# rubengooj/stvo-pl

Measured on AMD Instinct MI355X. Metric: stereo frames/s (match+optimizePose), higher is better.
Workload: dtype u8/fp4+f64; 1 GPU; BASELINE configs[2]: KITTI-00-shaped stereo with points + lines (ORB + LBD rows), grid-windowed stereo match (points and lines) + f2f brute-force mutual-NNR match (points and lines) + full GN optimizePose (config_kitti.yaml), device-resident per-frame pipeline; the streams cycle through the 8 sequence ids / 3 KITTI calibrations of configs[4] (sequence s on rank s mod G); streams_per_gpu=3072, parallelism=seq-shard x1

## Files before the change

### stvo-pl_amd/csrc/pose_block.h

```cpp
#pragma once
#include <type_traits>

#include "kernels.h"
#include "pose_math.h"

namespace stvo {

namespace {

constexpr int ACT_CONTINUE = 0, ACT_BREAK = 1, ACT_FAIL = 2;

struct PoseSh {
    double DT[16];
    double DT0[16];
    double DT1[16];
    double DTr[16];
    double cov[36];
    double eig[6];
    double H[36];
    double g[6];
    double err, err_prev, err_out, lambda;
    double s_p, s_l;
    unsigned long long xchg[2];
    int action, good, n_inl_p, n_inl_l, n_m_p, n_m_l, evals, itmp;
};

__device__ __forceinline__ void store_total(PoseSh* sh, int k, double s) {
    if (k < 21) {
        const int i = (k >= 6) + (k >= 11) + (k >= 15) + (k >= 18) + (k >= 20), j = k - (i * (13 - i)) / 2 + i;
        sh->H[i * 6 + j] = s;
        sh->H[j * 6 + i] = s;
    } else if (k < 27) {
        sh->g[k - 21] = s;
    } else {
        sh->err = s / (double)(sh->n_inl_l + sh->n_inl_p);
    }
}

template <int NWORK>
struct BlockOps {
    static constexpr int NW = NWORK;
    static constexpr int WTHREADS = NWORK * 64;

    template <int CTRL, int ROW_MASK>
    static __device__ __forceinline__ double dpp_add(double v) {
        const long long b = __double_as_longlong(v);
        const int lo = __builtin_amdgcn_update_dpp(0, (int)(b & 0xFFFFFFFFll), CTRL, ROW_MASK, 0xf, true);
        const int hi = __builtin_amdgcn_update_dpp(0, (int)(b >> 32), CTRL, ROW_MASK, 0xf, true);
        return v + __longlong_as_double(((long long)hi << 32) | (unsigned long long)(unsigned)lo);
    }
    static __device__ __forceinline__ double wave_sum_lane63(double v) {
        v = dpp_add<0x111, 0xf>(v);
        v = dpp_add<0x112, 0xf>(v);
        v = dpp_add<0x114, 0xf>(v);
        v = dpp_add<0x118, 0xf>(v);
        v = dpp_add<0x142, 0xa>(v);
        v = dpp_add<0x143, 0xc>(v);
        return v;
    }
    static __device__ __forceinline__ double wave_sum(double v) {
#pragma unroll
        for (int off = 32; off > 0; off >>= 1) v += __shfl_xor(v, off, 64);
        return v;
    }
    static __device__ __forceinline__ int wave_sum_i(int v) {
#pragma unroll
        for (int off = 32; off > 0; off >>= 1) v += __shfl_xor(v, off, 64);
        return v;
    }

    static __device__ __forceinline__ double fold32(double a, double b) {
        const unsigned long long ab = (unsigned long long)__double_as_longlong(a), bb = (unsigned long long)__double_as_longlong(b);
        const auto lo = __builtin_amdgcn_permlane32_swap((unsigned)ab, (unsigned)bb, false, false);
        const auto hi = __builtin_amdgcn_permlane32_swap((unsigned)(ab >> 32), (unsigned)(bb >> 32), false, false);
        return __longlong_as_double((long long)(((unsigned long long)hi[0] << 32) | lo[0])) +
               __longlong_as_double((long long)(((unsigned long long)hi[1] << 32) | lo[1]));
    }
    static __device__ __forceinline__ double fold16(double a, double b) {
        const unsigned long long ab = (unsigned long long)__double_as_longlong(a), bb = (unsigned long long)__double_as_longlong(b);
        const auto lo = __builtin_amdgcn_permlane16_swap((unsigned)ab, (unsigned)bb, false, false);
        const auto hi = __builtin_amdgcn_permlane16_swap((unsigned)(ab >> 32), (unsigned)(bb >> 32), false, false);
        return __longlong_as_double((long long)(((unsigned long long)hi[0] << 32) | lo[0])) +
               __longlong_as_double((long long)(((unsigned long long)hi[1] << 32) | lo[1]));
    }

    template <bool W>
    static __device__ __forceinline__ void sum28_fold(double* acc, double (*red)[28], bool sc = false) {
        const int lane = threadIdx.x & 63, wv = W ? (int)(threadIdx.x >> 6) : NW;
        if (W || sc) {
            double s14[14], s7[7];
#pragma unroll
            for (int k = 0; k < 14; ++k) s14[k] = fold32(acc[k], acc[14 + k]);
// ... 39 lines not shown
            }
        }
        __syncthreads();
#pragma unroll
        for (int k = 0; k < N; ++k) {
            double s = red[0][k];
#pragma unroll
            for (int w = 1; w < NW; ++w) s += red[w][k];
            out[k] = s;
        }
        __syncthreads();
    }

    template <bool W>
    static __device__ __forceinline__ int sum_int(int v, int* ired, bool sc = false) {
        const int lane = threadIdx.x & 63, wv = W ? (int)(threadIdx.x >> 6) : NW;
        if (W || sc) {
            const int s = wave_sum_i(v);
            if (lane == 0) ired[wv] = s;
        }
        __syncthreads();
        int t = 0;
#pragma unroll
        for (int w = 0; w < NW; ++w) t += ired[w];
        if (sc) t += ired[NW];
        __syncthreads();
        return t;
    }

    template <bool W>
    static __device__ __forceinline__ void sum_int4(const int* v, double (*red)[28], int* out, bool sc = false) {
        const int lane = threadIdx.x & 63, wv = W ? (int)(threadIdx.x >> 6) : NW;
        if (W || sc) {
#pragma unroll
            for (int k = 0; k < 4; ++k) {
                const int t = wave_sum_i(v[k]);
                if (lane == 0) reinterpret_cast<int*>(&red[wv][0])[k] = t;
            }
        }
        __syncthreads();
#pragma unroll
        for (int k = 0; k < 4; ++k) {
            int t = 0;
#pragma unroll
            for (int w = 0; w < NW; ++w) t += reinterpret_cast<const int*>(&red[w][0])[k];
            if (sc) t += reinterpret_cast<const int*>(&red[NW][0])[k];
            out[k] = t;
        }
    }

    static constexpr int HIST_W = 260;
    static constexpr int SEL_HW = 64, SEL_PART = 6 * SEL_HW;
    static_assert(SEL_PART * 4 % 8 == 0 && SEL_PART + 8 * (NWORK + 1) <= 2 * HIST_W, "selection scratch");

    static __device__ __forceinline__ int wave_incl_scan_i(int v) {
        v += __builtin_amdgcn_update_dpp(0, v, 0x111, 0xf, 0xf, true);
        v += __builtin_amdgcn_update_dpp(0, v, 0x112, 0xf, 0xf, true);
        v += __builtin_amdgcn_update_dpp(0, v, 0x114, 0xf, 0xf, true);
        v += __builtin_amdgcn_update_dpp(0, v, 0x118, 0xf, 0xf, true);
        v += __builtin_amdgcn_update_dpp(0, v, 0x142, 0xa, 0xf, true);
        v += __builtin_amdgcn_update_dpp(0, v, 0x143, 0xc, 0xf, true);
        return v;
    }
    static __device__ __forceinline__ void sel_scan(const unsigned* h, int kk, int& bin, int& below, int& cnt) {
        const int lane = threadIdx.x & 63;
        const unsigned w = h[lane];
        const int c0 = (int)(w & 0xFFFFu), c1 = (int)(w >> 16), sum = c0 + c1;
        const int incl = wave_incl_scan_i(sum), excl = incl - sum;
        const unsigned long long hit = __ballot(excl <= kk && kk < incl);
        const int L = hit ? __builtin_ctzll(hit) : 0;
        const bool up = kk >= excl + c0;
        bin = __builtin_amdgcn_readlane(2 * lane + (up ? 1 : 0), L);
        below = __builtin_amdgcn_readlane(excl + (up ? c0 : 0), L);
        cnt = __builtin_amdgcn_readlane(up ? c1 : c0, L);
    }
    template <int N, typename K, typename KeyFn>
    static __device__ __forceinline__ void sel_and_or(KeyFn&& key, unsigned mask, unsigned long long* part) {
        K k_and = ~(K)0, k_or = 0;
#pragma unroll
        for (int k = 0; k < N; ++k)
            if ((mask >> k) & 1u) {
                const K kv = key(k);
                k_and &= kv;
                k_or |= kv;
            }
        auto dpp_step = [&](auto ctrl_c, auto rmask_c) {
            constexpr int CTRL = decltype(ctrl_c)::value, RM = decltype(rmask_c)::value;
            const unsigned alo = (unsigned)k_and, ahi = (unsigned)((unsigned long long)k_and >> 32);
            const unsigned olo = (unsigned)k_or, ohi = (unsigned)((unsigned long long)k_or >> 32);
            const unsigned a0 = (unsigned)__builtin_amdgcn_update_dpp((int)alo, (int)alo, CTRL, RM, 0xf, false);
            const unsigned a1 = (unsigned)__builtin_amdgcn_update_dpp((int)ahi, (int)ahi, CTRL, RM, 0xf, false);
            const unsigned o0 = (unsigned)__builtin_amdgcn_update_dpp((int)olo, (int)olo, CTRL, RM, 0xf, false);
            const unsigned o1 = (unsigned)__builtin_amdgcn_update_dpp((int)ohi, (int)ohi, CTRL, RM, 0xf, false);
            k_and &= (K)(((unsigned long long)a1 << 32) | a0);
            k_or |= (K)(((unsigned long long)o1 << 32) | o0);
        };
        using std::integral_constant;
        dpp_step(integral_constant<int, 0x111>{}, integral_constant<int, 0xf>{});
        dpp_step(integral_constant<int, 0x112>{}, integral_constant<int, 0xf>{});
        dpp_step(integral_constant<int, 0x114>{}, integral_constant<int, 0xf>{});
        dpp_step(integral_constant<int, 0x118>{}, integral_constant<int, 0xf>{});
        dpp_step(integral_constant<int, 0x142>{}, integral_constant<int, 0xa>{});
        dpp_step(integral_constant<int, 0x143>{}, integral_constant<int, 0xc>{});
        if ((threadIdx.x & 63) == 63) {
            part[0] = (unsigned long long)k_and;
            part[1] = (unsigned long long)k_or;
        }
    }

    template <int NA, int NB, bool W, typename K, int BITS, typename KeyA, typename KeyB>
    static __device__ __forceinline__ void select2(KeyA&& ka, unsigned ma, int ktha, bool acta, KeyB&& kb, unsigned mb, int kthb, bool actb,
                                                   unsigned* S, unsigned long long* xchg, int& rot, K& outa, K& outb, bool sc = false) {
        static_assert(BITS == 32 || BITS == 64, "32- or 64-bit keys");
        const int tid = threadIdx.x, wv = tid >> 6;
        const bool own_b = W ? !sc : sc;
        constexpr bool PFA = BITS == 64 && NA >= 8, PFB = BITS == 64 && NB >= 8;
        K anda = 0, ora = ~(K)0, andb = 0, orb = ~(K)0;
        if (PFA || PFB) {
            unsigned long long* part = reinterpret_cast<unsigned long long*>(S + SEL_PART);
            if (W) {
                if (PFA) sel_and_or<NA, K>(ka, ma, part + 4 * wv);
                if (PFB && !sc) sel_and_or<NB, K>(kb, mb, part + 4 * wv + 2);
            }
            __syncthreads();
            unsigned long long a0 = ~0ull, o0 = 0ull, a1 = ~0ull, o1 = 0ull;
#pragma unroll
            for (int w = 0; w < NWORK; ++w) {
                if (PFA) { a0 &= part[4 * w]; o0 |= part[4 * w + 1]; }
                if (PFB) { a1 &= part[4 * w + 2]; o1 |= part[4 * w + 3]; }
            }
            if (PFA) { anda = (K)a0; ora = (K)o0; }
            if (PFB && !sc) { andb = (K)a1; orb = (K)o1; }
        }
        auto top_bit = [](K differ) -> int {
            return differ == 0 ? -1 : (BITS - 1) - (BITS == 64 ? __clzll((unsigned long long)differ) : __clz((unsigned)differ));
        };
        K pa = anda, pb = andb;
        int kka = ktha, kkb = kthb;
        int hia = acta ? top_bit(anda ^ ora) : -1, hib = actb ? top_bit(andb ^ orb) : -1;
        bool penda = false, pendb = false;
        auto count = [&](auto n_c, auto&& key, unsigned mask, K prefix, int hi, int lo, unsigned* h) {
            constexpr int N = decltype(n_c)::value;
#pragma unroll
            for (int k = 0; k < N; ++k) {
                const K kv = key(k);
                const K diff = kv ^ prefix;
                const bool same = hi + 1 >= BITS ? true : (diff >> (hi + 1 >= BITS ? 0 : hi + 1)) == 0;
                const unsigned bin = (unsigned)((kv >> lo) & 127);
                if (((mask >> k) & 1u) && same) atomicAdd(&h[bin >> 1], 1u << (16 * (bin & 1u)));
            }
        };
        auto decide = [&](auto n_c, bool own, auto&& key, unsigned mask, const unsigned* h, K& prefix, int& kk, int& hi, int lo, bool& pend,
                          unsigned long long* mail) {
            constexpr int N = decltype(n_c)::value;
            int bin, below, cnt;
            sel_scan(h, kk, bin, below, cnt);
            prefix = (prefix & ~((K)127 << lo)) | ((K)bin << lo);
            kk -= below;
            hi = lo - 1;
            if (cnt == 1 && lo > 0) {
                if (own) {
#pragma unroll
                    for (int k = 0; k < N; ++k) {
                        const K kv = key(k);
                        if (((mask >> k) & 1u) && ((kv ^ prefix) >> lo) == 0) *mail = (unsigned long long)kv;
                    }
                }
                pend = true;
                hi = -1;
            }
        };
        using std::integral_constant;
        while (hia >= 0 || hib >= 0) {
            const int loa = hia >= 6 ? hia - 6 : 0, lob = hib >= 6 ? hib - 6 : 0;
            unsigned* const ha = S + rot * SEL_HW;
            unsigned* const hb = S + (3 + rot) * SEL_HW;
            if (W && hia >= 0) count(integral_constant<int, NA>{}, ka, ma, pa, hia, loa, ha);
            if (own_b && hib >= 0) count(integral_constant<int, NB>{}, kb, mb, pb, hib, lob, hb);
            __syncthreads();
            if (W && tid < 2 * SEL_HW) {
                const int rc = rot == 0 ? 2 : rot - 1;
                S[((tid >> 6) * 3 + rc) * SEL_HW + (tid & 63)] = 0u;
            }
            if (hia >= 0) decide(integral_constant<int, NA>{}, W, ka, ma, ha, pa, kka, hia, loa, penda, xchg);
            if (hib >= 0) decide(integral_constant<int, NB>{}, own_b, kb, mb, hb, pb, kkb, hib, lob, pendb, xchg + 1);
            rot = rot == 2 ? 0 : rot + 1;
        }
        __syncthreads();
        if (penda) pa = (K)xchg[0];
        if (pendb) pb = (K)xchg[1];
        if (acta) outa = pa;
        if (actb) outb = pb;
    }

    template <int NA, int NB, bool W>
    static __device__ __forceinline__ void mad_sigma2(const double* va, unsigned ma, int na, const double* vb, unsigned mb, int nb, unsigned* S,
                                                      unsigned long long* xchg, int& rot, double& sa, double& sb, bool sc = false) {
        sa = 0.0;
        sb = 0.0;
        const bool acta = na != 0, actb = nb != 0;
        if (!acta && !actb) return;
        auto image = [](double v) -> unsigned long long {
            const unsigned long long b = (unsigned long long)__double_as_longlong(v);
            return (b >> 63) ? ~b : (b | 0x8000000000000000ull);
        };
        auto value = [](unsigned long long k) -> double {
            return __longlong_as_double((long long)((k >> 63) ? (k & 0x7FFFFFFFFFFFFFFFull) : ~k));
        };
        unsigned long long ra = 0ull, rb = 0ull;
        select2<NA, NB, W, unsigned long long, 64>([&](int k) { return image(va[k]); }, ma, na / 2, acta, [&](int k) { return image(vb[k]); }, mb,
                                                   nb / 2, actb, S, xchg, rot, ra, rb, sc);
        const double meda = value(ra), medb = value(rb);
        unsigned qa = 0u, qb = 0u;
        select2<NA, NB, W, unsigned, 32>([&](int k) { return __float_as_uint(fabsf((float)(va[k] - meda))); }, ma, na / 2, acta,
                                         [&](int k) { return __float_as_uint(fabsf((float)(vb[k] - medb))); }, mb, nb / 2, actb, S, xchg, rot, qa, qb, sc);
        if (acta) sa = 1.4826 * (double)__uint_as_float(qa);
        if (actb) sb = 1.4826 * (double)__uint_as_float(qb);
    }

    template <int N, bool W>
    static __device__ __forceinline__ void sum_at(const double* v, double (*red)[28], int slot0, double* out, bool sc = false) {
        const int lane = threadIdx.x & 63, wv = W ? (int)(threadIdx.x >> 6) : NW;
        if (W || sc) {
#pragma unroll
            for (int k = 0; k < N; ++k) {
                const double s = wave_sum_lane63(v[k]);
                if (lane == 63) red[wv][slot0 + k] = s;
            }
        }
        __syncthreads();
#pragma unroll
        for (int k = 0; k < N; ++k) {
            double s = red[0][slot0 + k];
#pragma unroll
            for (int w = 1; w < NW; ++w) s += red[w][slot0 + k];
            if (sc) s += red[NW][slot0 + k];
            out[k] = s;
        }
    }

    template <int NA, int NB, bool W>
    static __device__ __forceinline__ void outlier_cut(const double* ra, unsigned ma, int na, bool do_a, const double* rb, unsigned mb, int nb,
                                                       bool do_b, double inlier_k, unsigned& inla, unsigned& inlb, unsigned* S,
                                                       unsigned long long* xchg, int& rot, double (*red)[28], int* cnt, bool sc = false) {
        const bool own_b = W ? !sc : sc;
        double sa, sb;
        mad_sigma2<NA, NB, W>(ra, do_a ? ma : 0u, do_a ? na : 0, rb, do_b ? mb : 0u, do_b ? nb : 0, S, xchg, rot, sa, sb, sc);
        double v[6] = {0.0, 0.0, 0.0, 0.0, 0.0, 0.0};
        if (W) {
#pragma unroll
            for (int k = 0; k < NA; ++k)
                if (do_a && ((ma >> k) & 1u)) {
                    if (ra[k] < 2.0 * sa) {
                        v[0] += ra[k];
                        v[1] += 1.0;
                    }
                    v[2] += ra[k];
                }
        }
        if (own_b) {
#pragma unroll
            for (int k = 0; k < NB; ++k)
                if (do_b && ((mb >> k) & 1u)) {
                    if (rb[k] < 2.0 * sb) {
                        v[3] += rb[k];
                        v[4] += 1.0;
                    }
                    v[5] += rb[k];
// ... 147 lines not shown
#pragma unroll
        for (int i = 0; i < 16; ++i) DT[i] = sh->DT[i];
        pm::step_pose(DT, inc);
#pragma unroll
        for (int i = 0; i < 16; ++i) sh->DT[i] = DT[i];
    }
    if (norm3(inc) < min_error_change && norm3(inc + 3) < min_error_change) {
        sh->action = ACT_BREAK;
        return;
    }
    sh->err_prev = err;
    sh->action = ACT_CONTINUE;
}

__device__ __forceinline__ void t0_cov_from_H(PoseSh* sh, double* ws) {
    double H[36], Hi[36];
#pragma unroll
    for (int i = 0; i < 36; ++i) H[i] = sh->H[i];
    if (pm::inverse6_spd(H, Hi)) {
#pragma unroll
        for (int i = 0; i < 36; ++i) sh->cov[i] = Hi[i];
    } else {
#pragma unroll 1
        for (int i = 0; i < 36; ++i) ws[i] = sh->H[i];
        pm::inverse6_mem(ws, sh->cov);
    }
}

__device__ __forceinline__ void t0_is_good(PoseSh* sh, const double* DT, double err) {
    double C[36], w[6];
#pragma unroll
    for (int i = 0; i < 36; ++i) C[i] = sh->cov[i];
    pm::eig6_ql(C, w);
#pragma unroll
    for (int i = 0; i < 6; ++i) sh->eig[i] = w[i];
    sh->good = pm::is_good_solution(DT, w, err) ? 1 : 0;
}

__device__ __forceinline__ void t0_is_good_fast(PoseSh* sh, const double* DT, double err) {
    if (err < 0.0 || err > 1.0 || !pm::all_finite16(DT)) {
        sh->good = 0;
        return;
    }
    double C[36];
#pragma unroll
    for (int i = 0; i < 36; ++i) C[i] = sh->cov[i];
    if (pm::spd_unit_certificate(C) == 1) {
        sh->good = 1;
        return;
    }
    t0_is_good(sh, DT, err);
}

__device__ __forceinline__ void t0_commit(PoseSh* sh, stvo_pose_result* out, int status, int path, int it0, int it1, bool lazy_eig = false,
                                          double* next_T = nullptr) {
    bool eig_pending = false;
    if (lazy_eig) {
        double C[36];
#pragma unroll
        for (int i = 0; i < 36; ++i) C[i] = sh->cov[i];
        if (sh->err_out < 0.0 || sh->err_out > 1.0 || !pm::all_finite16(sh->DT)) {
            sh->good = 0;
        } else if (pm::spd_unit_certificate(C) == 1) {
            sh->good = 1;
            eig_pending = true;
        } else {
            t0_is_good(sh, sh->DT, sh->err_out);
        }
    } else {
        t0_is_good(sh, sh->DT, sh->err_out);
    }
    double DT[16];
#pragma unroll
    for (int i = 0; i < 16; ++i) {
        DT[i] = sh->DT[i];
        out->T_opt[i] = DT[i];
    }
    out->err_opt = sh->err_out;
    if (sh->good && !pm::is_identity16(DT)) {
        double Ti[16], x[6], T[16];
        pm::inverse_se3(DT, Ti);
        pm::logmap_se3(Ti, x);
        pm::expmap_se3(x, T);
#pragma unroll
        for (int i = 0; i < 16; ++i) out->T[i] = T[i];
        if (next_T) {
            const bool fin = pm::all_finite16(T);
#pragma unroll
            for (int i = 0; i < 16; ++i) next_T[i] = fin ? T[i] : ((i % 5 == 0) ? 1.0 : 0.0);
        }
#pragma unroll
        for (int i = 0; i < 36; ++i) out->cov[i] = sh->cov[i];
#pragma unroll
        for (int i = 0; i < 6; ++i) out->cov_eig[i] = eig_pending ? 0.0 : sh->eig[i];
        if (eig_pending) path |= PATH_EIG_PENDING;
        out->err = sh->err_out;
    } else {
#pragma unroll
        for (int i = 0; i < 16; ++i) out->T[i] = (i % 5 == 0) ? 1.0 : 0.0;
        if (next_T) {
#pragma unroll
            for (int i = 0; i < 16; ++i) next_T[i] = (i % 5 == 0) ? 1.0 : 0.0;
        }
#pragma unroll
        for (int i = 0; i < 36; ++i) out->cov[i] = 0.0;
#pragma unroll
        for (int i = 0; i < 6; ++i) out->cov_eig[i] = 0.0;
        out->err = -1.0;
        if (status == STVO_POSE_OK) status = STVO_POSE_REJECTED;
    }
    out->status = status;
    out->path = path;
    out->iters[0] = it0;
    out->iters[1] = it1;
    out->n_matched_pt = sh->n_m_p;
    out->n_matched_ls = sh->n_m_l;
    out->n_inliers_pt = sh->n_inl_p;
    out->n_inliers_ls = sh->n_inl_l;
}

}
}
```

### stvo-pl_amd/csrc/pose_kernel2p.hip

```cpp
#include <cstdlib>

#include <map>
#include <mutex>
#include <utility>
#include <vector>

#include "pose_block.h"

namespace stvo {
namespace {

__device__ __forceinline__ double uni(double v) {
    const long long b = __double_as_longlong(v);
    const int lo = __builtin_amdgcn_readfirstlane((int)(b & 0xFFFFFFFFll)), hi = __builtin_amdgcn_readfirstlane((int)(b >> 32));
    return __longlong_as_double(((long long)hi << 32) | (unsigned long long)(unsigned)lo);
}

struct PointRec2 {
    double X, Y, Z, ox, oy, q;
};

constexpr bool POSE2P_PRIO = true;

struct PoseFlow {
// ... 54 lines not shown
            if (stage != 0) {
                it1 = evals;
                break;
            }
            it0 = evals;
            tq2 = tick();
            if (w0) {
#pragma unroll
                for (int i = 0; i < 16; ++i) sh->DT1[i] = sh->DT[i];
                t0_is_good_fast(sh, sh->DT1, sh->err_out);
            }
            __syncthreads();
            tprof[2] += tick() - tq2;
            if (sh->good) {
                path |= STVO_PATH_STAGE1_GOOD;
                tq2 = tick();
                remove_outliers();
                tprof[3] += tick() - tq2;
                if (sh->n_inl_p + sh->n_inl_l >= prm().min_features) {
                    path |= STVO_PATH_REFINED;
                    stage = 1;
                } else {
                    if (w0) pm::identity4(sh->DT);
                    status = STVO_POSE_FEW_INLIERS_AFTER;
                    __syncthreads();
                    break;
                }
            } else {
                path |= STVO_PATH_ROBUST_FALLBACK;
                stage = 2;
                alg = 1;
            }
            max_it = prm().max_iters_ref;
            if (w0) {
#pragma unroll
                for (int i = 0; i < 16; ++i) sh->DT[i] = sh->DT0[i];
            }
            __syncthreads();
        }
    } else {
        if (w0) pm::identity4(sh->DT);
        status = STVO_POSE_FEW_INLIERS_BEFORE;
        __syncthreads();
    }

    return PoseFlow{status, path, it0, it1};
}

template <int NW, bool PROF>
__global__ __launch_bounds__(NW * 64, 2) void pose2p_kernel(PoseArgs a, const int k_lds, double2* arena, const size_t arena_pair) {
    constexpr int BLOCK = NW * 64;
    constexpr int PPT = (STVO_POSE_MAX_POINTS + BLOCK - 1) / BLOCK;
    constexpr int LPT = (STVO_POSE_MAX_LINES + BLOCK - 1) / BLOCK;
    using Ops = BlockOps<NW>;
    extern __shared__ double2 s_pl[];
    __shared__ __align__(16) int s_hist[2][Ops::HIST_W];
    __shared__ double s_red[NW][28];
    __shared__ int s_ired[NW];
    __shared__ PoseSh s_sh;
    PoseSh* sh = &s_sh;
    const int f = blockIdx.x, tid = threadIdx.x, lane = tid & 63, wv = tid >> 6;
    const bool w0 = wv == 0;
    const bool t0 = tid == 0;
    constexpr bool prof = PROF;
    long long tprof[5] = {0, 0, 0, 0, 0};
    long long wprof[3] = {0, 0, 0}, wave_busy = 0;
    auto tick = [&]() -> long long {
        if constexpr (PROF) return (long long)__builtin_readcyclecounter();
        else return 0ll;
    };
    const long long t_begin = tick();
    const stvo_cam cam_f = a.cams ? a.cams[f] : a.cam;
    const pm::Cam5 cam{cam_f.fx, cam_f.fy, cam_f.cx, cam_f.cy};
    const stvo_opt_params prm = a.prm;
    const double inv_homog = 1.0 / prm.homog_th;

    unsigned pmatched = 0u, pinl = 0u;
    const int n_prev_p = a.n_prev_pts != nullptr ? min(a.n_prev_pts[f], a.max_pts) : 0;
    const size_t pbase = (size_t)f * a.max_pts;
    int jj[PPT];
    {
        int init[PPT];
#pragma unroll
        for (int k = 0; k < PPT; ++k) {
            const int i = tid + k * BLOCK;
            const int ic = i < n_prev_p ? i : 0;
            jj[k] = a.m12p ? a.m12p[pbase + ic] : ic;
            init[k] = a.init_inl_p ? a.init_inl_p[pbase + ic] : 1;
        }
#pragma unroll
        for (int k = 0; k < PPT; ++k) {
            const int i = tid + k * BLOCK;
            if (i < n_prev_p && jj[k] >= 0) {
                pmatched |= 1u << k;
                if (init[k] != 0) pinl |= 1u << k;
            } else {
                jj[k] = 0;
            }
        }
    }
    unsigned lmatched = 0u, linl = 0u;
    const int n_prev_l = (a.n_prev_lines != nullptr && a.max_lines > 0) ? a.n_prev_lines[f] : 0;
    const size_t lbase = (size_t)f * a.max_lines;
    const int li0 = BLOCK - 1 - tid;
    int jl[LPT];
    {
        int initl[LPT];
#pragma unroll
        for (int k = 0; k < LPT; ++k) {
            const int li = li0 + k * BLOCK;
            const int lc = (li < n_prev_l && li < a.max_lines) ? li : 0;
            jl[k] = (a.m12l && a.max_lines > 0) ? a.m12l[lbase + lc] : lc;
            initl[k] = (a.init_inl_l && a.max_lines > 0) ? a.init_inl_l[lbase + lc] : 1;
        }
#pragma unroll
        for (int k = 0; k < LPT; ++k) {
            const int li = li0 + k * BLOCK;
            if (li < n_prev_l && li < a.max_lines && jl[k] >= 0) {
                lmatched |= 1u << k;
                if (initl[k] != 0) linl |= 1u << k;
            } else {
                jl[k] = 0;
            }
        }
    }

    unsigned* const sel = reinterpret_cast<unsigned*>(&s_hist[0][0]);
    int sel_rot = 0;
    for (int i = tid; i < 2 * Ops::HIST_W; i += BLOCK) sel[i] = 0u;
    const int n_m_p = Ops::template sum_int<true>(__popc(pmatched), s_ired);
    const int n_m_l = Ops::template sum_int<true>(__popc(lmatched), s_ired);
    auto launder = [](int v) -> int {
        asm volatile("" : "+v"(v));
        return v;
    };
    double2* ar = arena + (size_t)f * arena_pair;
    double2* ar_l = ar + (size_t)PPT * 3 * BLOCK;
    unsigned arena_mask = pmatched;
    for (int i = 0; i < k_lds; ++i) arena_mask &= arena_mask - 1u;
    const unsigned lds_mask = pmatched & ~arena_mask;
    auto ordinal = [&](int k) -> int { return __popc(pmatched & ((1u << k) - 1u)); };
    auto load_point_lds = [&](int k) -> PointRec2 {
        const int r = launder(ordinal(k));
        const double2* q = s_pl + (size_t)(r * 3) * BLOCK + tid;
        const double2 v0 = q[0], v1 = q[BLOCK], v2 = q[2 * BLOCK];
        PointRec2 rec;
        rec.X = v0.x; rec.Y = v0.y; rec.Z = v1.x; rec.ox = v1.y; rec.oy = v2.x; rec.q = v2.y;
        return rec;
    };
    auto load_point_arena = [&](int k) -> PointRec2 {
        const int r = launder(ordinal(k));
        const double2* q = ar + (size_t)(r * 3) * BLOCK + tid;
        const double2 v0 = q[0], v1 = q[BLOCK], v2 = q[2 * BLOCK];
        PointRec2 rec;
        rec.X = v0.x; rec.Y = v0.y; rec.Z = v1.x; rec.ox = v1.y; rec.oy = v2.x; rec.q = v2.y;
        return rec;
    };
    auto load_point = [&](int k) -> PointRec2 { return ((lds_mask >> k) & 1u) ? load_point_lds(k) : load_point_arena(k); };
    auto load_line = [&](int k) -> pm::LineRec {
        const int r = launder(__popc(lmatched & ((1u << k) - 1u)));
        const double2* q = ar_l + (size_t)(r * 7) * BLOCK + tid;
        pm::LineRec L;
        const double2 v0 = q[0], v1 = q[BLOCK], v2 = q[2 * BLOCK], v3 = q[3 * BLOCK], v4 = q[4 * BLOCK], v5 = q[5 * BLOCK], v6 = q[6 * BLOCK];
        L.sP[0] = v0.x; L.sP[1] = v0.y; L.sP[2] = v1.x; L.eP[0] = v1.y; L.eP[1] = v2.x; L.eP[2] = v2.y;
        L.le[0] = v3.x; L.le[1] = v3.y; L.le[2] = v4.x; L.spl[0] = v4.y; L.spl[1] = v5.x; L.epl[0] = v5.y; L.epl[1] = v6.x;
        L.sigma2 = v6.y;
        return L;
    };
    constexpr int STAGE_CH = PPT < 8 ? PPT : 8;
#pragma unroll
    for (int k0 = 0; k0 < PPT; k0 += STAGE_CH) {
        PointRec2 rec[STAGE_CH];
#pragma unroll
        for (int c = 0; c < STAGE_CH; ++c) {
            const int k = k0 + c;
            if (k >= PPT) continue;
            const int ik = tid + k * BLOCK;
            const size_t i = pbase + (size_t)(ik < n_prev_p ? ik : 0), j = pbase + (size_t)jj[k];
            rec[c].X = a.prev_P[i * 3 + 0];
            rec[c].Y = a.prev_P[i * 3 + 1];
            rec[c].Z = a.prev_P[i * 3 + 2];
            rec[c].q = a.prev_s2p[i];
// ... 157 lines not shown
    };

    if (a.eval_only) {
        evaluate(a.eval_robust != 0);
        if (w0) {
            if (t0) {
                double* o = a.eval_out + (size_t)f * 44;
#pragma unroll
                for (int i = 0; i < 36; ++i) o[i] = sh->H[i];
#pragma unroll
                for (int i = 0; i < 6; ++i) o[36 + i] = sh->g[i];
                o[42] = sh->err;
                o[43] = (double)(sh->n_inl_p + sh->n_inl_l);
            }
        }
        return;
    }

    auto remove_outliers = [&]() {
        double DT[12];
        pose_sgpr(sh->DT1, DT);
        double resp[PPT], resl[LPT];
#pragma unroll
        for (int k = 0; k < PPT; ++k) {
            resp[k] = 0.0;
            if (prm.has_points && ((pmatched >> k) & 1u)) {
                const PointRec2 r = load_point(k);
                resp[k] = pm::point_residual(DT, cam, r.X, r.Y, r.Z, r.ox, r.oy) * r.q;
            }
        }
#pragma unroll
        for (int k = 0; k < LPT; ++k) {
            resl[k] = 0.0;
            if (prm.has_lines && ((lmatched >> k) & 1u)) {
                const pm::LineRec L = load_line(k);
                resl[k] = pm::line_residual(DT, cam, L) * L.sigma2;
            }
        }
        int cnt[2];
        Ops::template outlier_cut<PPT, LPT, true>(resp, pmatched, sh->n_m_p, prm.has_points != 0, resl, lmatched, sh->n_m_l, prm.has_lines != 0,
                                                  prm.inlier_k, pinl, linl, sel, sh->xchg, sel_rot, s_red, cnt);
        if (w0) {
            if (prm.has_points) sh->n_inl_p = cnt[0];
            if (prm.has_lines) sh->n_inl_l = cnt[1];
        }
        __syncthreads();
    };

    const PoseFlow fl = optimize_pose_flow(sh, [&]() -> const stvo_opt_params& { return prm; }, w0, evaluate, remove_outliers, tick, tprof, &s_red[0][0]);
    const int status = fl.status, path = fl.path, it0 = fl.it0, it1 = fl.it1;

    {
        const long long tq3 = tick();
        if (t0) t0_commit(sh, a.results + f, status, path, it0, it1, false, a.next_T ? a.next_T + (size_t)f * 16 : nullptr);
        tprof[2] += tick() - tq3;
    }
    if (prof && t0) {
        tprof[4] = tick() - t_begin;
#pragma unroll
        for (int i = 0; i < 5; ++i) a.prof_out[(size_t)f * 16 + i] = tprof[i];
#pragma unroll
        for (int i = 0; i < 3; ++i) a.prof_out[(size_t)f * 16 + 5 + i] = wprof[i];
    }
    if (prof && lane == 0 && (wv < 6 || wv == NW - 1)) a.prof_out[(size_t)f * 16 + 8 + (wv < 6 ? wv : 7)] = wave_busy;
    if (prof && t0) a.prof_out[(size_t)f * 16 + 14] = t_prologue;

    if (a.inl_p_out) {
        const size_t base = (size_t)f * a.max_pts;
#pragma unroll
        for (int k = 0; k < PPT; ++k) {
            const int i = tid + k * BLOCK;
            if (i < a.max_pts) a.inl_p_out[base + i] = ((pmatched >> k) & 1u) ? (int)((pinl >> k) & 1u) : -1;
        }
    }
    if (a.inl_l_out && a.max_lines > 0) {
#pragma unroll
        for (int k = 0; k < LPT; ++k) {
            const int li = li0 + k * BLOCK;
            if (li < a.max_lines) a.inl_l_out[(size_t)f * a.max_lines + li] = ((lmatched >> k) & 1u) ? (int)((linl >> k) & 1u) : -1;
        }
    }
}

template <int I, int N, typename F>
__device__ __forceinline__ void static_for(F&& f) {
    if constexpr (I < N) {
        f(std::integral_constant<int, I>{});
        static_for<I + 1, N>(f);
    }
}

typedef float f4_native __attribute__((ext_vector_type(4)));
template <int N>
struct RecRegs {
    f4_native a0;
    double b0;
    RecRegs<N - 1> rest;
    template <int R>
    __device__ __forceinline__ f4_native& a() {
        if constexpr (R == 0) return a0;
        else return rest.template a<R - 1>();
    }
    template <int R>
    __device__ __forceinline__ double& b() {
        if constexpr (R == 0) return b0;
        else return rest.template b<R - 1>();
    }
};
template <>
struct RecRegs<0> {};

template <int NW>
constexpr int pose2c_planes() {
    return NW == 2 ? 12 : STVO_POSE_MAX_POINTS / (NW * 64);
}

struct CompactRec {
    float4 uvo;
    double bd;
    double q;
};

__device__ __noinline__ CompactRec pose2c_fetch_slow(const float4* prev_rc, const float4* curr_rc, const int32_t* m12p, size_t pbase,
                                                     int tid, int block, unsigned pmatched, int r, double cam_b, double level_scale) {
    unsigned m = pmatched;
    for (int i = 0; i < r; ++i) m &= m - 1u;
    const size_t i = pbase + (size_t)(tid + __builtin_ctz(m) * block);
    const size_t j = m12p ? pbase + (size_t)m12p[i] : i;
    const float4 p = prev_rc[i], c = curr_rc[j];
    CompactRec rec;
    rec.uvo = make_float4(p.x, p.y, c.x, c.y);
    rec.bd = cam_b / (double)p.z;
    rec.q = sqrt(pm::level_sigma2((int)p.w, level_scale));
    return rec;
}

template <int NW, bool PROF>
__global__ __launch_bounds__(NW * 64, 2) void pose2c_kernel(PoseArgs a_by_value, double2* arena, const size_t arena_pair) {
    (void)a_by_value;
    typedef const PoseArgs __attribute__((address_space(4))) KArgs;
    KArgs* const kargs = (KArgs*)__builtin_amdgcn_kernarg_segment_ptr();
    auto ka = [&]() -> KArgs& {
        KArgs* p = kargs;
        asm volatile("" : "+s"(p));
        return *p;
    };

    constexpr int BLOCK = NW * 64;
    constexpr int PPT = (STVO_POSE_MAX_POINTS + BLOCK - 1) / BLOCK;
    constexpr int LPT = (STVO_POSE_MAX_LINES + BLOCK - 1) / BLOCK;
    constexpr int KL = pose2c_planes<NW>();
    constexpr bool HAS_REG = KL < PPT;
    static_assert(KL <= PPT && PPT <= 16, "4-bit levels of 16 ordinals in one 64-bit word");
    using Ops = BlockOps<NW>;
    extern __shared__ float4 s_ra[];
    double* const s_rb = reinterpret_cast<double*>(s_ra + KL * BLOCK);
    __shared__ __align__(16) int s_hist[2][Ops::HIST_W];
    __shared__ double s_red[NW][28];
    __shared__ int s_ired[NW];
    __shared__ PoseSh s_sh;
    PoseSh* sh = &s_sh;
    const int f = blockIdx.x, tid = threadIdx.x, lane = tid & 63, wv = tid >> 6;
    const bool w0 = wv == 0, t0 = tid == 0;
    long long rprof[3] = {0, 0, 0};
    long long tprof[5] = {0, 0, 0, 0, 0};
    long long wprof[3] = {0, 0, 0}, wave_busy = 0;
    auto tick = [&]() -> long long {
        if constexpr (PROF) return (long long)__builtin_readcyclecounter();
        else return 0ll;
    };
    const long long t_begin = tick();
    if (blockIdx.x == 0 && threadIdx.x == 0 && ka().start_flag)
        __hip_atomic_store(ka().start_flag, ka().start_value, __ATOMIC_RELEASE, __HIP_MEMORY_SCOPE_AGENT);
    stvo_cam cam_f;
    if (ka().cams) {
        cam_f = ka().cams[f];
    } else {
        cam_f.fx = ka().cam.fx; cam_f.fy = ka().cam.fy; cam_f.cx = ka().cam.cx; cam_f.cy = ka().cam.cy; cam_f.b = ka().cam.b;
    }
    const pm::Cam5 cam{cam_f.fx, cam_f.fy, cam_f.cx, cam_f.cy};
    const double cam_b = cam_f.b;
    const double homog_th = ka().prm.homog_th, inv_homog = 1.0 / homog_th;

    unsigned pmatched = 0u, pinl = 0u;
    const int n_prev_p = ka().n_prev_pts != nullptr ? min(ka().n_prev_pts[f], ka().max_pts) : 0;
    const size_t pbase = (size_t)f * ka().max_pts;
    int jj[PPT];
    {
        int init[PPT];
        const int last = ka().max_pts - 1;
#pragma unroll
        for (int k = 0; k < PPT; ++k) {
            const int i = tid + k * BLOCK;
            const int ic = i < last ? i : last;
            jj[k] = ka().m12p ? ka().m12p[pbase + ic] : ic;
            init[k] = ka().init_inl_p ? ka().init_inl_p[pbase + ic] : 1;
        }
#pragma unroll
        for (int k = 0; k < PPT; ++k) {
            const int i = tid + k * BLOCK;
            if (i < n_prev_p && jj[k] >= 0) {
                pmatched |= 1u << k;
                if (init[k] != 0) pinl |= 1u << k;
            } else {
                jj[k] = 0;
            }
        }
    }
    unsigned lmatched = 0u, linl = 0u;
    const int n_prev_l = (ka().n_prev_lines != nullptr && ka().max_lines > 0) ? ka().n_prev_lines[f] : 0;
    const size_t lbase = (size_t)f * ka().max_lines;
    const int li0 = BLOCK - 1 - tid;
    int jl[LPT];
    {
        int initl[LPT];
#pragma unroll
        for (int k = 0; k < LPT; ++k) {
            const int li = li0 + k * BLOCK;
            const int lc = (li < n_prev_l && li < ka().max_lines) ? li : 0;
            jl[k] = (ka().m12l && ka().max_lines > 0) ? ka().m12l[lbase + lc] : lc;
            initl[k] = (ka().init_inl_l && ka().max_lines > 0) ? ka().init_inl_l[lbase + lc] : 1;
        }
#pragma unroll
        for (int k = 0; k < LPT; ++k) {
            const int li = li0 + k * BLOCK;
            if (li < n_prev_l && li < ka().max_lines && jl[k] >= 0) {
                lmatched |= 1u << k;
                if (initl[k] != 0) linl |= 1u << k;
            } else {
                jl[k] = 0;
            }
        }
    }
    const int n_mine = __popc(pmatched);
    unsigned* const sel = reinterpret_cast<unsigned*>(&s_hist[0][0]);
    int sel_rot = 0;
    for (int i = tid; i < 2 * Ops::HIST_W; i += BLOCK) sel[i] = 0u;
    const int n_m_p = Ops::template sum_int<true>(n_mine, s_ired);
    const int n_m_l = Ops::template sum_int<true>(__popc(lmatched), s_ired);

    const unsigned m_o = n_mine >= 32 ? 0xFFFFFFFFu : ((1u << n_mine) - 1u);
    unsigned inl_o = 0u, slow_o = 0u;
    unsigned long long lv = 0ull;
    float4 xa = make_float4(0.f, 0.f, 0.f, 0.f);
    double xb = 1.0;
    {
        int r = 0;
        constexpr int STAGE_CH = PPT;
#pragma unroll
        for (int k0 = 0; k0 < PPT; k0 += STAGE_CH) {
            float4 pv[STAGE_CH], cv[STAGE_CH];
#pragma unroll
            for (int c = 0; c < STAGE_CH; ++c) {
                const int k = k0 + c;
                if (k >= PPT) continue;
                const int ik = tid + k * BLOCK;
                pv[c] = ka().prev_rc[pbase + (size_t)(ik < n_prev_p ? ik : 0)];
                cv[c] = ka().curr_rc[pbase + (size_t)jj[k]];
            }
#pragma unroll
            for (int c = 0; c < STAGE_CH; ++c) {
                const int k = k0 + c;
                if (k >= PPT) continue;
                if ((pmatched >> k) & 1u) {
                    const int level = (int)pv[c].w;
                    const bool in_tab = level >= 0 && level < STVO_POSE_QTAB - 1;
                    const float4 av = make_float4(pv[c].x, pv[c].y, cv[c].x, cv[c].y);
                    const double bd = cam_b / (double)pv[c].z;
                    if (r < KL) {
                        s_ra[r * BLOCK + tid] = av;
                        s_rb[r * BLOCK + tid] = bd;
                    } else if (HAS_REG && r == KL) {
                        xa = av;
                        xb = bd;
                    }
                    lv |= (unsigned long long)(in_tab ? level : STVO_POSE_QTAB - 1) << (4 * r);
                    if (r > (HAS_REG ? KL : KL - 1) || !in_tab) slow_o |= 1u << r;
                    if ((pinl >> k) & 1u) inl_o |= 1u << r;
                    ++r;
                }
            }
            __builtin_amdgcn_sched_barrier(0);
        }
    }
    int n_trip = n_mine < KL ? n_mine : KL;
#pragma unroll
    for (int off = 32; off > 0; off >>= 1) n_trip = max(n_trip, __shfl_xor(n_trip, off, 64));
    n_trip = __builtin_amdgcn_readfirstlane(n_trip);
    bool dealt = false;
    unsigned inl_w = 0u;
// ... 202 lines not shown
            const int o = __shfl_up(incl, off, 64);
            if (lane >= off) incl += o;
        }
        const int n_slow = Ops::template sum_int<true>(__popc(inl_o & slow_o), s_ired);
        if (lane == 63) s_ired[wv] = incl;
        __syncthreads();
        int base = incl - c, total = 0;
#pragma unroll
        for (int w = 0; w < NW; ++w) {
            const int cw = s_ired[w];
            if (w < wv) base += cw;
            total += cw;
        }
        __syncthreads();
        if (n_slow != 0 || total > KL * BLOCK) return;
        RecRegs<HAS_REG ? KL + 1 : KL> regs;
        auto take = [&](auto rc) {
            constexpr int R = decltype(rc)::value;
            if constexpr (R < KL) {
                regs.template a<R>() = *reinterpret_cast<const f4_native*>(&s_ra[R * BLOCK + tid]);
                regs.template b<R>() = s_rb[R * BLOCK + tid];
            } else {
                regs.template a<R>() = f4_native{xa.x, xa.y, xa.z, xa.w};
                regs.template b<R>() = xb;
            }
        };
        static_for<0, HAS_REG ? KL + 1 : KL>(take);
        __syncthreads();
        {
            int g = base;
            auto put = [&](auto rc) {
                constexpr int R = decltype(rc)::value;
                if ((mov >> R) & 1u) {
                    *reinterpret_cast<f4_native*>(&s_ra[g]) = regs.template a<R>();
                    s_rb[g] = regs.template b<R>();
                    s_lvb[g] = (unsigned char)((lv >> (4 * R)) & 15u);
                    ++g;
                }
            };
            static_for<0, HAS_REG ? KL + 1 : KL>(put);
        }
        __syncthreads();
        const int n_hold = tid < total ? (total - tid + BLOCK - 1) / BLOCK : 0;
        unsigned long long lvn = 0ull;
#pragma unroll
        for (int r = 0; r < KL; ++r)
            if (r < n_hold) lvn |= (unsigned long long)s_lvb[r * BLOCK + tid] << (4 * r);
        lv = lvn;
        inl_w = n_hold > 0 ? ((1u << n_hold) - 1u) : 0u;
        dealt = true;
        const int first = wv * 64;
        n_trip = first < total ? (total - first + BLOCK - 1) / BLOCK : 0;
        __syncthreads();
        for (int i = tid; i < 2 * Ops::HIST_W; i += BLOCK) sel[i] = 0u;
        __syncthreads();
    };

    auto remove_outliers = [&]() {
        double DT[12];
        pose_sgpr(sh->DT1, DT);
        const bool do_p = ka().prm.has_points != 0, do_l = ka().prm.has_lines != 0;
        const long long tr0 = tick();
        double resp[PPT], resl[LPT];
        residuals(DT, do_p ? m_o : 0u, true, resp);
#pragma unroll
        for (int k = 0; k < LPT; ++k) {
            resl[k] = 0.0;
            if (do_l && ((lmatched >> k) & 1u)) {
                const pm::LineRec L = load_line(k);
                resl[k] = pm::line_residual(DT, cam, L) * L.sigma2;
            }
        }
        const long long tr1 = tick();
        int cnt[2];
        Ops::template outlier_cut<PPT, LPT, true>(resp, m_o, sh->n_m_p, do_p, resl, lmatched, sh->n_m_l, do_l, ka().prm.inlier_k, inl_o, linl, sel,
                                                  sh->xchg, sel_rot, s_red, cnt);
        if (w0) {
            if (do_p) sh->n_inl_p = cnt[0];
            if (do_l) sh->n_inl_l = cnt[1];
        }
        __syncthreads();
        const long long tr2 = tick();
        compact_inliers();
        rprof[0] += tr1 - tr0;
        rprof[1] += tr2 - tr1;
        rprof[2] += tick() - tr2;
    };

    const PoseFlow fl = optimize_pose_flow(sh, [&]() -> const stvo_opt_params __attribute__((address_space(4)))& { return ka().prm; }, w0, evaluate,
                                           remove_outliers, tick, tprof, &s_red[0][0]);

    {
        const long long tq3 = tick();
        if (t0) t0_commit(sh, ka().results + f, fl.status, fl.path, fl.it0, fl.it1, false, ka().next_T ? ka().next_T + (size_t)f * 16 : nullptr);
        tprof[2] += tick() - tq3;
    }
    if (PROF && t0) {
        tprof[4] = tick() - t_begin;
#pragma unroll
        for (int i = 0; i < 5; ++i) ka().prof_out[(size_t)f * 16 + i] = tprof[i];
#pragma unroll
        for (int i = 0; i < 3; ++i) ka().prof_out[(size_t)f * 16 + 5 + i] = wprof[i];
        ka().prof_out[(size_t)f * 16 + 14] = t_prologue;
#pragma unroll
        for (int i = 0; i < 3; ++i) ka().prof_out[(size_t)f * 16 + 10 + i] = rprof[i];
    }
    if (PROF && lane == 0 && (wv < 6 || wv == NW - 1)) ka().prof_out[(size_t)f * 16 + 8 + (wv < 6 ? wv : 7)] = wave_busy;

    if (ka().inl_p_out) {
        const size_t base = (size_t)f * ka().max_pts;
#pragma unroll
        for (int k = 0; k < PPT; ++k) {
            const int i = tid + k * BLOCK;
            const int r = __popc(pmatched & ((1u << k) - 1u));
            if (i < ka().max_pts) ka().inl_p_out[base + i] = ((pmatched >> k) & 1u) ? (int)((inl_o >> r) & 1u) : -1;
        }
    }
    if (ka().inl_l_out && ka().max_lines > 0) {
#pragma unroll
        for (int k = 0; k < LPT; ++k) {
            const int li = li0 + k * BLOCK;
            if (li < ka().max_lines) ka().inl_l_out[(size_t)f * ka().max_lines + li] = ((lmatched >> k) & 1u) ? (int)((linl >> k) & 1u) : -1;
        }
    }
}

struct ArenaBuf {
    double2* dev = nullptr;
    size_t bytes = 0;
    int users = 0;
    std::vector<void*> retired;
};

std::mutex g_arena_mu;
std::map<std::pair<int, hipStream_t>, ArenaBuf> g_arenas;

double2* arena_ptr(hipStream_t s, size_t bytes) {
    int dev = 0;
    if (hipGetDevice(&dev) != hipSuccess) return nullptr;
    std::lock_guard<std::mutex> lk(g_arena_mu);
    ArenaBuf& b = g_arenas[std::make_pair(dev, s)];
    if (b.bytes < bytes || !b.dev) {
        if (b.dev) b.retired.push_back(b.dev);
        b.dev = nullptr;
        b.bytes = 0;
        if (hipMalloc((void**)&b.dev, bytes > 256 ? bytes : 256) != hipSuccess) return nullptr;
        b.bytes = bytes;
// ... 78 lines not shown
```

Baseline: 1.389 million frame-pairs/s.

## Use per-lane packed radix counts for median selection and split final commit across waves

Adds a lane-counting radix-select variant (select2_lp) that packs 8-bit digit counters per lane, reduces them with DPP scans into small per-wave rows, and picks the bin with a ballot. This replaces the shared-memory histogram with atomics and avoids the histogram-zeroing passes. It also overlaps the 6x6 covariance eigen-decomposition on a second wave with the solution verdict and output commit on wave 0, and skips the high-word DPP ops for 32-bit keys. The cost is 4-bit digits instead of 6, which means more selection rounds, each ending in a block barrier.

```diff
diff --git a/stvo-pl_amd/csrc/pose_block.h b/stvo-pl_amd/csrc/pose_block.h
--- a/stvo-pl_amd/csrc/pose_block.h
+++ b/stvo-pl_amd/csrc/pose_block.h
@@ -37,7 +37,7 @@
     }
 }
 
-template <int NWORK>
+template <int NWORK, bool LANE_COUNT = false>
 struct BlockOps {
     static constexpr int NW = NWORK;
     static constexpr int WTHREADS = NWORK * 64;
@@ -183,6 +183,8 @@
     static constexpr int HIST_W = 260;
     static constexpr int SEL_HW = 64, SEL_PART = 6 * SEL_HW;
     static_assert(SEL_PART * 4 % 8 == 0 && SEL_PART + 8 * (NWORK + 1) <= 2 * HIST_W, "selection scratch");
+    static constexpr int LP_ROWS = 8 * NWORK;
+    static_assert(LP_ROWS + 2 * 2 * NWORK * 8 <= 2 * HIST_W, "selection scratch");
 
     static __device__ __forceinline__ int wave_incl_scan_i(int v) {
         v += __builtin_amdgcn_update_dpp(0, v, 0x111, 0xf, 0xf, true);
@@ -217,14 +219,19 @@
             }
         auto dpp_step = [&](auto ctrl_c, auto rmask_c) {
             constexpr int CTRL = decltype(ctrl_c)::value, RM = decltype(rmask_c)::value;
-            const unsigned alo = (unsigned)k_and, ahi = (unsigned)((unsigned long long)k_and >> 32);
-            const unsigned olo = (unsigned)k_or, ohi = (unsigned)((unsigned long long)k_or >> 32);
+            const unsigned alo = (unsigned)k_and, olo = (unsigned)k_or;
             const unsigned a0 = (unsigned)__builtin_amdgcn_update_dpp((int)alo, (int)alo, CTRL, RM, 0xf, false);
-            const unsigned a1 = (unsigned)__builtin_amdgcn_update_dpp((int)ahi, (int)ahi, CTRL, RM, 0xf, false);
             const unsigned o0 = (unsigned)__builtin_amdgcn_update_dpp((int)olo, (int)olo, CTRL, RM, 0xf, false);
-            const unsigned o1 = (unsigned)__builtin_amdgcn_update_dpp((int)ohi, (int)ohi, CTRL, RM, 0xf, false);
-            k_and &= (K)(((unsigned long long)a1 << 32) | a0);
-            k_or |= (K)(((unsigned long long)o1 << 32) | o0);
+            if constexpr (sizeof(K) == 8) {
+                const unsigned ahi = (unsigned)((unsigned long long)k_and >> 32), ohi = (unsigned)((unsigned long long)k_or >> 32);
+                const unsigned a1 = (unsigned)__builtin_amdgcn_update_dpp((int)ahi, (int)ahi, CTRL, RM, 0xf, false);
+                const unsigned o1 = (unsigned)__builtin_amdgcn_update_dpp((int)ohi, (int)ohi, CTRL, RM, 0xf, false);
+                k_and &= (K)(((unsigned long long)a1 << 32) | a0);
+                k_or |= (K)(((unsigned long long)o1 << 32) | o0);
+            } else {
+                k_and &= (K)a0;
+                k_or |= (K)o0;
+            }
         };
         using std::integral_constant;
         dpp_step(integral_constant<int, 0x111>{}, integral_constant<int, 0xf>{});
@@ -316,6 +323,128 @@
             if (hia >= 0) decide(integral_constant<int, NA>{}, W, ka, ma, ha, pa, kka, hia, loa, penda, xchg);
             if (hib >= 0) decide(integral_constant<int, NB>{}, own_b, kb, mb, hb, pb, kkb, hib, lob, pendb, xchg + 1);
             rot = rot == 2 ? 0 : rot + 1;
+        }
+        __syncthreads();
+        if (penda) pa = (K)xchg[0];
+        if (pendb) pb = (K)xchg[1];
+        if (acta) outa = pa;
+        if (actb) outb = pb;
+    }
+
+    template <typename K>
+    static __device__ __forceinline__ K uni_key(K v) {
+        const unsigned lo = (unsigned)__builtin_amdgcn_readfirstlane((int)(unsigned)v);
+        if constexpr (sizeof(K) == 8) {
+            const unsigned hi = (unsigned)__builtin_amdgcn_readfirstlane((int)(unsigned)((unsigned long long)v >> 32));
+            return (K)(((unsigned long long)hi << 32) | lo);
+        } else {
+            return (K)lo;
+        }
+    }
+    template <int N, typename K, int BITS, typename KeyFn>
+    static __device__ __forceinline__ void lp_count(KeyFn&& key, unsigned mask, K prefix, int hi, int lo, unsigned* row) {
+        static_assert(N <= 255, "8-bit lane counters");
+        unsigned c[4] = {0u, 0u, 0u, 0u};
+#pragma unroll
+        for (int k = 0; k < N; ++k) {
+            const K kv = key(k);
+            const bool same = hi + 1 >= BITS ? true : ((kv ^ prefix) >> (hi + 1 >= BITS ? 0 : hi + 1)) == 0;
+            const unsigned d = (unsigned)(kv >> lo) & 15u;
+            const unsigned inc = (((mask >> k) & 1u) && same) ? 1u << (8 * (d & 3u)) : 0u;
+            const unsigned q = d >> 2;
+#pragma unroll
+            for (int j = 0; j < 4; ++j) c[j] += q == (unsigned)j ? inc : 0u;
+        }
+        unsigned w[8];
+#pragma unroll
+        for (int j = 0; j < 4; ++j) {
+            w[2 * j] = (c[j] & 0xFFu) | ((c[j] & 0xFF00u) << 8);
+            w[2 * j + 1] = ((c[j] >> 16) & 0xFFu) | ((c[j] >> 8) & 0xFF0000u);
+        }
+#pragma unroll
+        for (int j = 0; j < 8; ++j) w[j] = (unsigned)wave_incl_scan_i((int)w[j]);
+        if ((threadIdx.x & 63) == 63) {
+            *reinterpret_cast<uint4*>(row) = make_uint4(w[0], w[1], w[2], w[3]);
+            *reinterpret_cast<uint4*>(row + 4) = make_uint4(w[4], w[5], w[6], w[7]);
+        }
+    }
+    template <int NA, int NB, typename K, int BITS, typename KeyA, typename KeyB>
+    static __device__ __forceinline__ void select2_lp(KeyA&& ka, unsigned ma, int ktha, bool acta, KeyB&& kb, unsigned mb, int kthb, bool actb,
+                                                      unsigned* S, unsigned long long* xchg, K& outa, K& outb) {
+        static_assert(BITS == 32 || BITS == 64, "32- or 64-bit keys");
+        const int lane = threadIdx.x & 63, wv = threadIdx.x >> 6;
+        K pa = 0, pb = 0;
+        int hia = -1, hib = -1;
+        {
+            unsigned long long* part = reinterpret_cast<unsigned long long*>(S);
+            if (acta) sel_and_or<NA, K>(ka, ma, part + 4 * wv);
+            if (actb) sel_and_or<NB, K>(kb, mb, part + 4 * wv + 2);
+            __syncthreads();
+            unsigned long long a0 = ~0ull, o0 = 0ull, a1 = ~0ull, o1 = 0ull;
+#pragma unroll
+            for (int w = 0; w < NWORK; ++w) {
+                a0 &= part[4 * w]; o0 |= part[4 * w + 1];
+                a1 &= part[4 * w + 2]; o1 |= part[4 * w + 3];
+            }
+            auto top_bit = [](K differ) -> int {
+                return differ == 0 ? -1 : (BITS - 1) - (BITS == 64 ? __clzll((unsigned long long)differ) : __clz((unsigned)differ));
+            };
+            if (acta) {
+                pa = uni_key<K>((K)a0);
+                hia = top_bit(uni_key<K>((K)(a0 ^ o0)));
+            }
+            if (actb) {
+                pb = uni_key<K>((K)a1);
+                hib = top_bit(uni_key<K>((K)(a1 ^ o1)));
+            }
+        }
+        int kka = ktha, kkb = kthb;
+        bool penda = false, pendb = false;
+        auto decide = [&](auto n_c, auto&& key, unsigned mask, int bin, int below, int cnt, K& prefix, int& kk, int& hi, int lo, bool& pend,
+                          unsigned long long* mail) {
+            constexpr int N = decltype(n_c)::value;
+            prefix = (prefix & ~((K)15 << lo)) | ((K)bin << lo);
+            kk -= below;
+            hi = lo - 1;
+            if (cnt == 1 && lo > 0) {
+#pragma unroll
+                for (int k = 0; k < N; ++k) {
+                    const K kv = key(k);
+                    if (((mask >> k) & 1u) && ((kv ^ prefix) >> lo) == 0) *mail = (unsigned long long)kv;
+                }
+                pend = true;
+                hi = -1;
+            }
+        };
+        using std::integral_constant;
+        int buf = 0;
+        while (hia >= 0 || hib >= 0) {
+            const int loa = hia >= 3 ? hia - 3 : 0, lob = hib >= 3 ? hib - 3 : 0;
+            unsigned* const rows = S + LP_ROWS + buf * (2 * NWORK * 8);
+            if (hia >= 0) lp_count<NA, K, BITS>(ka, ma, pa, hia, loa, rows + wv * 8);
+            if (hib >= 0) lp_count<NB, K, BITS>(kb, mb, pb, hib, lob, rows + (NWORK + wv) * 8);
+            __syncthreads();
+            const int setl = (lane >> 4) & 1, d = lane & 15;
+            const unsigned short* col = reinterpret_cast<const unsigned short*>(rows + setl * NWORK * 8) + d;
+            int cnt = 0;
+#pragma unroll
+            for (int w = 0; w < NWORK; ++w) cnt += (int)col[w * 16];
+            int incl = cnt;
+            incl += __builtin_amdgcn_update_dpp(0, incl, 0x111, 0xf, 0xf, true);
+            incl += __builtin_amdgcn_update_dpp(0, incl, 0x112, 0xf, 0xf, true);
+            incl += __builtin_amdgcn_update_dpp(0, incl, 0x114, 0xf, 0xf, true);
+            incl += __builtin_amdgcn_update_dpp(0, incl, 0x118, 0xf, 0xf, true);
+            const int excl = incl - cnt, kkl = setl ? kkb : kka;
+            const unsigned long long hit = __ballot(excl <= kkl && kkl < incl);
+            const unsigned hita = (unsigned)hit & 0xFFFFu, hitb = (unsigned)(hit >> 16) & 0xFFFFu;
+            const int La = hita ? __builtin_ctz(hita) : 0, Lb = 16 + (hitb ? __builtin_ctz(hitb) : 0);
+            if (hia >= 0)
+                decide(integral_constant<int, NA>{}, ka, ma, La, __builtin_amdgcn_readlane(excl, La), __builtin_amdgcn_readlane(cnt, La), pa, kka, hia,
+                       loa, penda, xchg);
+            if (hib >= 0)
+                decide(integral_constant<int, NB>{}, kb, mb, Lb - 16, __builtin_amdgcn_readlane(excl, Lb), __builtin_amdgcn_readlane(cnt, Lb), pb, kkb,
+                       hib, lob, pendb, xchg + 1);
+            buf ^= 1;
         }
         __syncthreads();
         if (penda) pa = (K)xchg[0];
@@ -339,12 +468,20 @@
             return __longlong_as_double((long long)((k >> 63) ? (k & 0x7FFFFFFFFFFFFFFFull) : ~k));
         };
         unsigned long long ra = 0ull, rb = 0ull;
-        select2<NA, NB, W, unsigned long long, 64>([&](int k) { return image(va[k]); }, ma, na / 2, acta, [&](int k) { return image(vb[k]); }, mb,
-                                                   nb / 2, actb, S, xchg, rot, ra, rb, sc);
+        auto keya = [&](int k) { return image(va[k]); };
+        auto keyb = [&](int k) { return image(vb[k]); };
+        if constexpr (LANE_COUNT) {
+            static_assert(W, "select2_lp: every wave is a worker");
+            select2_lp<NA, NB, unsigned long long, 64>(keya, ma, na / 2, acta, keyb, mb, nb / 2, actb, S, xchg, ra, rb);
+        } else {
+            select2<NA, NB, W, unsigned long long, 64>(keya, ma, na / 2, acta, keyb, mb, nb / 2, actb, S, xchg, rot, ra, rb, sc);
+        }
         const double meda = value(ra), medb = value(rb);
         unsigned qa = 0u, qb = 0u;
-        select2<NA, NB, W, unsigned, 32>([&](int k) { return __float_as_uint(fabsf((float)(va[k] - meda))); }, ma, na / 2, acta,
-                                         [&](int k) { return __float_as_uint(fabsf((float)(vb[k] - medb))); }, mb, nb / 2, actb, S, xchg, rot, qa, qb, sc);
+        auto deva = [&](int k) { return __float_as_uint(fabsf((float)(va[k] - meda))); };
+        auto devb = [&](int k) { return __float_as_uint(fabsf((float)(vb[k] - medb))); };
+        if constexpr (LANE_COUNT) select2_lp<NA, NB, unsigned, 32>(deva, ma, na / 2, acta, devb, mb, nb / 2, actb, S, xchg, qa, qb);
+        else select2<NA, NB, W, unsigned, 32>(deva, ma, na / 2, acta, devb, mb, nb / 2, actb, S, xchg, rot, qa, qb, sc);
         if (acta) sa = 1.4826 * (double)__uint_as_float(qa);
         if (actb) sb = 1.4826 * (double)__uint_as_float(qb);
     }
@@ -598,24 +735,8 @@
     t0_is_good(sh, DT, err);
 }
 
-__device__ __forceinline__ void t0_commit(PoseSh* sh, stvo_pose_result* out, int status, int path, int it0, int it1, bool lazy_eig = false,
-                                          double* next_T = nullptr) {
-    bool eig_pending = false;
-    if (lazy_eig) {
-        double C[36];
-#pragma unroll
-        for (int i = 0; i < 36; ++i) C[i] = sh->cov[i];
-        if (sh->err_out < 0.0 || sh->err_out > 1.0 || !pm::all_finite16(sh->DT)) {
-            sh->good = 0;
-        } else if (pm::spd_unit_certificate(C) == 1) {
-            sh->good = 1;
-            eig_pending = true;
-        } else {
-            t0_is_good(sh, sh->DT, sh->err_out);
-        }
-    } else {
-        t0_is_good(sh, sh->DT, sh->err_out);
-    }
+constexpr int EIG_NOW = 0, EIG_HOST = 1, EIG_LATER = 2;
+__device__ __forceinline__ bool t0_commit_outputs(PoseSh* sh, stvo_pose_result* out, int status, int path, int it0, int it1, int eig, double* next_T) {
     double DT[16];
 #pragma unroll
     for (int i = 0; i < 16; ++i) {
@@ -623,7 +744,8 @@
         out->T_opt[i] = DT[i];
     }
     out->err_opt = sh->err_out;
-    if (sh->good && !pm::is_identity16(DT)) {
+    const bool committed = sh->good && !pm::is_identity16(DT);
+    if (committed) {
         double Ti[16], x[6], T[16];
         pm::inverse_se3(DT, Ti);
         pm::logmap_se3(Ti, x);
@@ -637,9 +759,11 @@
         }
 #pragma unroll
         for (int i = 0; i < 36; ++i) out->cov[i] = sh->cov[i];
-#pragma unroll
-        for (int i = 0; i < 6; ++i) out->cov_eig[i] = eig_pending ? 0.0 : sh->eig[i];
-        if (eig_pending) path |= PATH_EIG_PENDING;
+        if (eig != EIG_LATER) {
+#pragma unroll
+            for (int i = 0; i < 6; ++i) out->cov_eig[i] = eig == EIG_HOST ? 0.0 : sh->eig[i];
+        }
+        if (eig == EIG_HOST) path |= PATH_EIG_PENDING;
         out->err = sh->err_out;
     } else {
 #pragma unroll
@@ -663,7 +787,67 @@
     out->n_matched_ls = sh->n_m_l;
     out->n_inliers_pt = sh->n_inl_p;
     out->n_inliers_ls = sh->n_inl_l;
-}
-
-}
-}
+    return committed;
+}
+
+__device__ __forceinline__ int t0_verdict_no_eig(const PoseSh* sh) {
+    if (sh->err_out < 0.0 || sh->err_out > 1.0 || !pm::all_finite16(sh->DT)) return 0;
+    double C[36];
+#pragma unroll
+    for (int i = 0; i < 36; ++i) C[i] = sh->cov[i];
+    return pm::spd_unit_certificate(C) == 1 ? 1 : -1;
+}
+
+__device__ __forceinline__ void t0_commit(PoseSh* sh, stvo_pose_result* out, int status, int path, int it0, int it1, bool lazy_eig = false,
+                                          double* next_T = nullptr) {
+    bool eig_pending = false;
+    if (lazy_eig) {
+        const int v = t0_verdict_no_eig(sh);
+        if (v < 0) {
+            t0_is_good(sh, sh->DT, sh->err_out);
+        } else {
+            sh->good = v;
+            eig_pending = v == 1;
+        }
+    } else {
+        t0_is_good(sh, sh->DT, sh->err_out);
+    }
+    t0_commit_outputs(sh, out, status, path, it0, it1, eig_pending ? EIG_HOST : EIG_NOW, next_T);
+}
+
+__device__ __forceinline__ void commit_two_waves(PoseSh* sh, stvo_pose_result* out, int status, int path, int it0, int it1, double* next_T) {
+    const int tid = threadIdx.x;
+    int verdict = 0;
+    bool committed = false;
+    if (tid == 0) {
+        verdict = t0_verdict_no_eig(sh);
+        if (verdict >= 0) {
+            sh->good = verdict;
+            committed = t0_commit_outputs(sh, out, status, path, it0, it1, EIG_LATER, next_T);
+        }
+    } else if (tid == 64) {
+        double C[36], w[6];
+#pragma unroll
+        for (int i = 0; i < 36; ++i) C[i] = sh->cov[i];
+        pm::eig6_ql(C, w);
+#pragma unroll
+        for (int i = 0; i < 6; ++i) sh->eig[i] = w[i];
+    }
+    __syncthreads();
+    if (tid == 0) {
+        double w[6];
+#pragma unroll
+        for (int i = 0; i < 6; ++i) w[i] = sh->eig[i];
+        if (verdict < 0) {
+            sh->good = pm::is_good_solution(sh->DT, w, sh->err_out) ? 1 : 0;
+            committed = t0_commit_outputs(sh, out, status, path, it0, it1, EIG_LATER, next_T);
+        }
+        if (committed) {
+#pragma unroll
+            for (int i = 0; i < 6; ++i) out->cov_eig[i] = w[i];
+        }
+    }
+}
+
+}
+}
diff --git a/stvo-pl_amd/csrc/pose_kernel2p.hip b/stvo-pl_amd/csrc/pose_kernel2p.hip
--- a/stvo-pl_amd/csrc/pose_kernel2p.hip
+++ b/stvo-pl_amd/csrc/pose_kernel2p.hip
@@ -130,7 +130,7 @@
     constexpr int BLOCK = NW * 64;
     constexpr int PPT = (STVO_POSE_MAX_POINTS + BLOCK - 1) / BLOCK;
     constexpr int LPT = (STVO_POSE_MAX_LINES + BLOCK - 1) / BLOCK;
-    using Ops = BlockOps<NW>;
+    using Ops = BlockOps<NW, true>;
     extern __shared__ double2 s_pl[];
     __shared__ __align__(16) int s_hist[2][Ops::HIST_W];
     __shared__ double s_red[NW][28];
@@ -205,7 +205,6 @@
 
     unsigned* const sel = reinterpret_cast<unsigned*>(&s_hist[0][0]);
     int sel_rot = 0;
-    for (int i = tid; i < 2 * Ops::HIST_W; i += BLOCK) sel[i] = 0u;
     const int n_m_p = Ops::template sum_int<true>(__popc(pmatched), s_ired);
     const int n_m_l = Ops::template sum_int<true>(__popc(lmatched), s_ired);
     auto launder = [](int v) -> int {
@@ -469,7 +468,7 @@
 
     {
         const long long tq3 = tick();
-        if (t0) t0_commit(sh, a.results + f, status, path, it0, it1, false, a.next_T ? a.next_T + (size_t)f * 16 : nullptr);
+        commit_two_waves(sh, a.results + f, status, path, it0, it1, a.next_T ? a.next_T + (size_t)f * 16 : nullptr);
         tprof[2] += tick() - tq3;
     }
     if (prof && t0) {
@@ -569,7 +568,7 @@
     constexpr int KL = pose2c_planes<NW>();
     constexpr bool HAS_REG = KL < PPT;
     static_assert(KL <= PPT && PPT <= 16, "4-bit levels of 16 ordinals in one 64-bit word");
-    using Ops = BlockOps<NW>;
+    using Ops = BlockOps<NW, true>;
     extern __shared__ float4 s_ra[];
     double* const s_rb = reinterpret_cast<double*>(s_ra + KL * BLOCK);
     __shared__ __align__(16) int s_hist[2][Ops::HIST_W];
@@ -652,7 +651,6 @@
     const int n_mine = __popc(pmatched);
     unsigned* const sel = reinterpret_cast<unsigned*>(&s_hist[0][0]);
     int sel_rot = 0;
-    for (int i = tid; i < 2 * Ops::HIST_W; i += BLOCK) sel[i] = 0u;
     const int n_m_p = Ops::template sum_int<true>(n_mine, s_ired);
     const int n_m_l = Ops::template sum_int<true>(__popc(lmatched), s_ired);
 
@@ -961,8 +959,6 @@
         const int first = wv * 64;
         n_trip = first < total ? (total - first + BLOCK - 1) / BLOCK : 0;
         __syncthreads();
-        for (int i = tid; i < 2 * Ops::HIST_W; i += BLOCK) sel[i] = 0u;
-        __syncthreads();
     };
 
     auto remove_outliers = [&]() {
@@ -1001,7 +997,7 @@
 
     {
         const long long tq3 = tick();
-        if (t0) t0_commit(sh, ka().results + f, fl.status, fl.path, fl.it0, fl.it1, false, ka().next_T ? ka().next_T + (size_t)f * 16 : nullptr);
+        commit_two_waves(sh, ka().results + f, fl.status, fl.path, fl.it0, fl.it1, ka().next_T ? ka().next_T + (size_t)f * 16 : nullptr);
         tprof[2] += tick() - tq3;
     }
     if (PROF && t0) {
```

After: 1.363 million frame-pairs/s. -1.9%, worse.
